# cg-tuwien/ppsurf

Hardware: AMD Instinct MI355X
Metric: occupancy query-points/sec @ res=257, 50NN (higher is better)
Workload: dtype f16x3

## Files before the change

### ppsurf_amd/csrc/pps_common.h

```cpp
#pragma once
#include <hip/hip_runtime.h>
#include <stdint.h>

typedef float f32x4 __attribute__((ext_vector_type(4)));

#define PPS_WAVE 64
#define PPS_OK 0
#define PPS_ERR_ARG 1
#define PPS_ERR_LAUNCH 2

#define PPS_SG_MFMA 0x008
#define PPS_SG_DSREAD 0x100
#define PPS_SG_VALU 0x002

namespace pps {

__device__ __forceinline__ int lane_id() { return threadIdx.x & 63; }

template <int CTRL>
__device__ __forceinline__ float dpp_mov(float v) {
    return __builtin_bit_cast(float, __builtin_amdgcn_update_dpp(0, __builtin_bit_cast(int, v), CTRL, 0xf, 0xf, true));
}
__device__ __forceinline__ float row16_max(float v) {
    v = fmaxf(v, dpp_mov<0xB1>(v));
    v = fmaxf(v, dpp_mov<0x4E>(v));
    v = fmaxf(v, dpp_mov<0x141>(v));
    v = fmaxf(v, dpp_mov<0x140>(v));
    return v;
}
__device__ __forceinline__ float row16_sum(float v) {
    v += dpp_mov<0xB1>(v);
    v += dpp_mov<0x4E>(v);
    v += dpp_mov<0x141>(v);
    v += dpp_mov<0x140>(v);
    return v;
}

__device__ __forceinline__ float max_raw(float a, float b) {
    float r;
    asm("v_max_f32 %0, %1, %2" : "=v"(r) : "v"(a), "v"(b));
    return r;
}

#define PPS_DPP4(OP, CTRL)                                                    \
    OP " %0, %0, %0 " CTRL " row_mask:0xf bank_mask:0xf bound_ctrl:1\n\t"      \
    OP " %1, %1, %1 " CTRL " row_mask:0xf bank_mask:0xf bound_ctrl:1\n\t"      \
    OP " %2, %2, %2 " CTRL " row_mask:0xf bank_mask:0xf bound_ctrl:1\n\t"      \
    OP " %3, %3, %3 " CTRL " row_mask:0xf bank_mask:0xf bound_ctrl:1\n\t"
__device__ __forceinline__ void row16_max4(float& a, float& b, float& c, float& d) {
    asm("s_nop 1\n\t" PPS_DPP4("v_max_f32_dpp", "quad_perm:[1,0,3,2]") PPS_DPP4("v_max_f32_dpp", "quad_perm:[2,3,0,1]")
        PPS_DPP4("v_max_f32_dpp", "row_half_mirror") PPS_DPP4("v_max_f32_dpp", "row_mirror")
        : "+v"(a), "+v"(b), "+v"(c), "+v"(d));
}
__device__ __forceinline__ void row16_sum4(float& a, float& b, float& c, float& d) {
    asm("s_nop 1\n\t" PPS_DPP4("v_add_f32_dpp", "quad_perm:[1,0,3,2]") PPS_DPP4("v_add_f32_dpp", "quad_perm:[2,3,0,1]")
        PPS_DPP4("v_add_f32_dpp", "row_half_mirror") PPS_DPP4("v_add_f32_dpp", "row_mirror")
        : "+v"(a), "+v"(b), "+v"(c), "+v"(d));
}
#undef PPS_DPP4

template <int CTRL>
__device__ __forceinline__ unsigned dpp_mov_u32(unsigned v) { return (unsigned)__builtin_amdgcn_update_dpp(0, (int)v, CTRL, 0xf, 0xf, true); }
__device__ __forceinline__ unsigned lane_xor_u32(unsigned v, int st, int lane) {
    switch (st) {
    case 1: return dpp_mov_u32<0xB1>(v);
    case 2: return dpp_mov_u32<0x4E>(v);
    case 4: return dpp_mov_u32<0x1B>(dpp_mov_u32<0x141>(v));
    case 8: return dpp_mov_u32<0x141>(dpp_mov_u32<0x140>(v));
    case 16: { const auto r = __builtin_amdgcn_permlane16_swap(v, v, false, false); return (lane & 16) ? r[0] : r[1]; }
    case 32: { const auto r = __builtin_amdgcn_permlane32_swap(v, v, false, false); return (lane & 32) ? r[0] : r[1]; }
    default: return (unsigned)__shfl_xor((int)v, st);
    }
}
__device__ __forceinline__ unsigned long long lane_xor_u64(unsigned long long v, int st, int lane) {
    return ((unsigned long long)lane_xor_u32((unsigned)(v >> 32), st, lane) << 32) | lane_xor_u32((unsigned)v, st, lane);
}

template <int CTRL>
__device__ __forceinline__ f32x4 dpp_mov4(f32x4 v) { return f32x4{dpp_mov<CTRL>(v.x), dpp_mov<CTRL>(v.y), dpp_mov<CTRL>(v.z), dpp_mov<CTRL>(v.w)}; }

template <int HALF, int CTRL>
__device__ __forceinline__ void butterfly_step(f32x4* v, bool upper) {
#pragma unroll
    for (int b = 0; b < HALF; ++b) {
        const f32x4 keep = upper ? v[b + HALF] : v[b];
        const f32x4 send = upper ? v[b] : v[b + HALF];
        v[b] = keep + dpp_mov4<CTRL>(send);
    }
}
__device__ __forceinline__ void rows16_sum_transposed(f32x4 (&v)[16], int lane) {
    butterfly_step<8, 0x128>(v, (lane & 8) != 0);
    butterfly_step<4, 0x141>(v, (lane & 4) != 0);
    butterfly_step<2, 0x4E>(v, (lane & 2) != 0);
// ... 209 lines not shown
template <int NF4, int NTHREADS>
__device__ __forceinline__ void chunk_copy_async(const f32x4* __restrict__ src, f32x4* dst) {
    unsigned lane_off = threadIdx.x * 16u;
    asm volatile("" : "+v"(lane_off));
    const int wave_base = threadIdx.x & ~63;
    const char* sbase = (const char*)src;
    asm volatile("" : "+s"(sbase));
#pragma unroll
    for (int i = 0; i < NF4; ++i) {
        f32x4* d = dst + i * NTHREADS + wave_base;
        const unsigned lds_addr = __builtin_amdgcn_readfirstlane((unsigned)(uintptr_t)d);
        const char* piece = sbase + (size_t)(i * NTHREADS * 16);
        asm volatile("s_mov_b32 m0, %0\n\tglobal_load_lds_dwordx4 %1, %2" : : "s"(lds_addr), "v"(lane_off), "s"(piece) : "memory", "m0");
    }
}
template <int NTHREADS>
__device__ __forceinline__ void chunk_copy_piece(const f32x4* __restrict__ src, f32x4* dst, int i) {
    unsigned lane_off = threadIdx.x * 16u;
    asm volatile("" : "+v"(lane_off));
    const int wave_base = threadIdx.x & ~63;
    const char* piece = (const char*)src + (size_t)i * (NTHREADS * 16);
    asm volatile("" : "+s"(piece));
    const unsigned lds_addr = __builtin_amdgcn_readfirstlane((unsigned)(uintptr_t)(dst + i * NTHREADS + wave_base));
    asm volatile("s_mov_b32 m0, %0\n\tglobal_load_lds_dwordx4 %1, %2" : : "s"(lds_addr), "v"(lane_off), "s"(piece) : "memory", "m0");
}
template <int NTHREADS, int NPIECES>
__device__ __forceinline__ void stream_lane_offsets(unsigned (&voff)[NPIECES]) {
#pragma unroll
    for (int i = 0; i < NPIECES; ++i) {
        voff[i] = threadIdx.x * 16u + (unsigned)i * (NTHREADS * 16u);
        asm volatile("" : "+v"(voff[i]));
    }
}
template <int NTHREADS>
__device__ __forceinline__ void chunk_copy_piece_at(const char* chunk, f32x4* dst, int i, unsigned voff) {
    const int wave_base = threadIdx.x & ~63;
    const unsigned lds_addr = __builtin_amdgcn_readfirstlane((unsigned)(uintptr_t)(dst + i * NTHREADS + wave_base));
    asm volatile("s_mov_b32 m0, %0\n\tglobal_load_lds_dwordx4 %1, %2" : : "s"(lds_addr), "v"(voff), "s"(chunk) : "memory", "m0");
}
__device__ __forceinline__ void stream_wait() {
    asm volatile("s_waitcnt vmcnt(0)" : : : "memory");
}

__device__ __forceinline__ void xcd_tile_range(int ntiles, int& first, int& count, int& stride) {
    const int nwg = gridDim.x;
    const int b = blockIdx.x;
    if ((nwg & 7) != 0 || nwg < 8) { first = b; stride = nwg; count = (ntiles > b) ? (ntiles - b + nwg - 1) / nwg : 0; return; }
    const int xcd = b & 7, slot = b >> 3, per = nwg >> 3;
    const int lo = (int)(((int64_t)ntiles * xcd) / 8), hi = (int)(((int64_t)ntiles * (xcd + 1)) / 8);
    first = lo + slot; stride = per;
    count = (hi - lo > slot) ? (hi - lo - slot + per - 1) / per : 0;
}

}
```

### ppsurf_amd/csrc/pps_decode.hip

```cpp
#include <cstdlib>
#include "pps_common.h"
#include "../../include/ppsurf_amd.h"

using namespace pps;

#ifndef NT
#define NT 256
#endif
#define NW (NT / 64)
#ifndef WG_PER_CU
#define WG_PER_CU (512 / NT)
#endif
#ifndef PPS_PRIO
#define PPS_PRIO 1
#endif
#ifndef PPS_PRIO_PN
#define PPS_PRIO_PN 1
#endif
#define CH4 2048

template <int CHUNK_F4_NEXT, int NTH = NT, class F>
__device__ __forceinline__ void stream_step(const f32x4* __restrict__ gnext, f32x4*& cur, f32x4*& nxt, F&& compute) {
    chunk_copy_async<CHUNK_F4_NEXT / NTH, NTH>(gnext, nxt);
    compute((const f32x4*)cur);
// ... 178 lines not shown
                    e[bb * 4 + r] = ev;
                    m4[bb][r] = mx;
                    s4[bb][r] = row16_sum(ev);
                }
            if (n < 4) {
                const f32x4 mm = (n == 0) ? m4[0] : (n == 1) ? m4[1] : (n == 2) ? m4[2] : m4[3];
                const f32x4 ss = (n == 0) ? s4[0] : (n == 1) ? s4[1] : (n == 2) ? s4[2] : s4[3];
                ((f32x4*)(msm + wave * 64))[4 * n + g] = mm;
                ((f32x4*)(mss + wave * 64))[4 * n + g] = ss;
            }
        }
        __syncthreads();
        {
            float mw[4], sw[4];
#pragma unroll
            for (int w2 = 0; w2 < 4; ++w2) { mw[w2] = msm[(wbase + w2) * 64 + lane]; sw[w2] = mss[(wbase + w2) * 64 + lane]; }
            const float M = fmaxf(fmaxf(mw[0], mw[1]), fmaxf(mw[2], mw[3]));
            float S = 0.f;
#pragma unroll
            for (int w2 = 0; w2 < 4; ++w2) S += sw[w2] * __expf(mw[w2] - M);
            f_l[wave * 64 + lane] = __expf(mw[wq] - M) / (64.f * S);
        }
        __syncthreads();
        float an = 0.f;
#pragma unroll
        for (int bb = 0; bb < 4; ++bb) {
            const f32x4 f4 = ((const f32x4*)(f_l + wave * 64))[4 * bb + g];
#pragma unroll
            for (int r = 0; r < 4; ++r) an += e[bb * 4 + r] * f4[r];
        }
        an += __shfl_xor(an, 16);
        an += __shfl_xor(an, 32);
#pragma unroll
        for (int bb = 0; bb < 16; ++bb) a[bb] *= an;
        rows16_sum_transposed(a, lane);
        ((f32x4*)(part + wave * 256))[4 * n + g] = a[0];
        __syncthreads();
        if (wq == 0 && qv) {
            f32x4 s = ((const f32x4*)(part + (wbase + 0) * 256))[lane];
            s += ((const f32x4*)(part + (wbase + 1) * 256))[lane];
            s += ((const f32x4*)(part + (wbase + 2) * 256))[lane];
            s += ((const f32x4*)(part + (wbase + 3) * 256))[lane];
            ((f32x4*)(pooled + qi * 256))[lane] = s;
        }
    }
}

#define IH_NT 512
#define IH_OB 2
#define IH_NW (IH_NT / 64)
#define IH_WG_PER_CU (512 / IH_NT)
#define IH_CH4 (CH4 * IH_OB / 2)
#define IH_NCH (32 / IH_OB + 4 / IH_OB)
#define IH_LDS_BYTES (2 * IH_CH4 * 16 + (IP_W_XYZ + IP_NBIAS + IH_NW * 64 * 3 + IH_NW * 256) * 4)

__global__ __launch_bounds__(IH_NT, 2) void interp_pool_f16x3_kernel(const float* __restrict__ G, const float* __restrict__ pts,
                                                                     const float* __restrict__ query, const int64_t* __restrict__ idx,
                                                                     int64_t Q, int k, const float* __restrict__ wxyz,
                                                                     const f32x4* __restrict__ w16, const float* __restrict__ bias,
                                                                     float* __restrict__ pooled, int* __restrict__ range) {
    float amax = 0.f;
    f32x4* buf0 = (f32x4*)pps_smem;
    f32x4* buf1 = buf0 + IH_CH4;
    float* xyz_l = (float*)(buf1 + IH_CH4);
    float* bias_l = xyz_l + IP_W_XYZ;
    float* msm = bias_l + IP_NBIAS;
    float* mss = msm + IH_NW * 64;
    float* f_l = mss + IH_NW * 64;
    float* part = f_l + IH_NW * 64;
    const f32x4* bias4 = (const f32x4*)bias_l;
    const f32x4* wg = w16;
    const int lane = lane_id(), wave = threadIdx.x >> 6, n = lane & 15, g = lane >> 4;

    lds_fill(xyz_l, wxyz, IP_W_XYZ);
    lds_fill(bias_l, bias, IP_NBIAS);
    stream_prologue<IH_CH4, IH_NT>(wg, buf0);
    stream_wait();
    __syncthreads();
    f32x4 *cur = buf0, *nxt = buf1;
    unsigned voff[IH_CH4 / IH_NT];
    stream_lane_offsets<IH_NT>(voff);
    const char* const wfirst = (const char*)wg;
    const char* snext = wfirst + (size_t)IH_CH4 * 16;

    const int ntiles = (int)((Q + IH_NW / 4 - 1) / (IH_NW / 4));
    int first, count, stride;
    xcd_tile_range(ntiles, first, count, stride);
    const int wq = wave & 3, wbase = wave & ~3;
    for (int it = 0; it < count; ++it) {
        const int64_t qi = (int64_t)(first + it * stride) * (IH_NW / 4) + (wave >> 2);
        const bool qv = qi < Q;
        const int64_t qc = qv ? qi : Q - 1;
        const int row = wq * 16 + n;
        const bool valid = row < k;
        const int64_t i = idx[qc * k + (valid ? row : 0)];

        HiLo x[8], y[8];
        {
            f32x4 a[16];
            const f32x4* grow = (const f32x4*)(G + i * 256) + g;
#pragma unroll
            for (int bb = 0; bb < 16; ++bb) a[bb] = grow[4 * bb];
            const float coord = (g < 3) ? (query[qc * 3 + g] - pts[i * 3 + g]) : 0.f;
            xyz_blocks<16>(coord, a, xyz_l, lane);
            relu_blocks<16>(a);
#pragma unroll
            for (int kb = 0; kb < 8; ++kb) x[kb] = split_f16_r(amax, a[2 * kb], a[2 * kb + 1]);
        }
        __builtin_amdgcn_s_setprio(PPS_PRIO);
#ifndef PPS_FCQ_PRODUCTS
#define PPS_FCQ_PRODUCTS 3
#endif
#define IH_STEP(LAST, IN, BIAS, ACTV, SINK) IH_STEP_NP(LAST, IN, BIAS, ACTV, SINK, 3)
#define IH_STEP_NP(LAST, IN, BIAS, ACTV, SINK, NPR)                                                                                   \
        {                                                                                                                             \
            stream_step_spread_at<IH_CH4, IH_NT>(snext, voff, cur, nxt, [&](const f32x4* w, auto&& piece) {                            \
                dense_blocks_f16x3_hook<8, IH_OB, ACTV, true, false, NPR>(IN, (const half8*)w, BIAS, lane, SINK,                       \
                                                    [&](int ob, int kb) { if (ob == 0 && (kb & 1) == 0) piece(kb >> 1); if (IH_CH4 / IH_NT > 4 && ob == 0 && (kb & 1)) piece(4 + (kb >> 1)); }); }); \
            snext = (LAST) ? wfirst : snext + (size_t)IH_CH4 * 16;                                                                     \
            asm volatile("" : "+s"(snext));                                      \
        }
#pragma unroll
        for (int c = 0; c < 16 / IH_OB; ++c)
            IH_STEP(false, x, bias4 + 4 * IH_OB * c, 1, ([&](int p, const f32x4& o0, const f32x4& o1) { y[IH_OB / 2 * c + p] = split_f16_r(amax, o0, o1); }));
#pragma unroll
        for (int c = 0; c < 16 / IH_OB; ++c)
            IH_STEP(false, y, bias4 + 64 + 4 * IH_OB * c, 1, ([&](int p, const f32x4& o0, const f32x4& o1) { x[IH_OB / 2 * c + p] = split_f16_r(amax, o0, o1); }));
        f32x4 b[4];
#pragma unroll
        for (int c = 0; c < 4 / IH_OB; ++c)
            IH_STEP_NP(c + 32 / IH_OB + 2 == IH_NCH, x, bias4 + 128 + 4 * IH_OB * c, 0,
                       ([&](int p, const f32x4& o0, const f32x4& o1) { b[IH_OB * c + 2 * p] = o0; b[IH_OB * c + 2 * p + 1] = o1; }), PPS_FCQ_PRODUCTS);
#undef IH_STEP
#undef IH_STEP_NP
        __builtin_amdgcn_s_setprio(0);
        float e[16];
        {
            f32x4 m4[4], s4[4];
#pragma unroll
            for (int bb = 0; bb < 4; ++bb) {
                float v[4], mx[4], sm[4];
#pragma unroll
                for (int r = 0; r < 4; ++r) mx[r] = v[r] = valid ? b[bb][r] : -INFINITY;
                row16_max4(mx[0], mx[1], mx[2], mx[3]);
#pragma unroll
                for (int r = 0; r < 4; ++r) {
                    const float ev = valid ? __expf(v[r] - mx[r]) : 0.f;
                    e[bb * 4 + r] = ev;
                    sm[r] = ev;
                }
                row16_sum4(sm[0], sm[1], sm[2], sm[3]);
                m4[bb] = f32x4{mx[0], mx[1], mx[2], mx[3]};
                s4[bb] = f32x4{sm[0], sm[1], sm[2], sm[3]};
            }
            if (n < 4) {
                const f32x4 mm = (n == 0) ? m4[0] : (n == 1) ? m4[1] : (n == 2) ? m4[2] : m4[3];
                const f32x4 ss = (n == 0) ? s4[0] : (n == 1) ? s4[1] : (n == 2) ? s4[2] : s4[3];
                ((f32x4*)(msm + wave * 64))[4 * n + g] = mm;
                ((f32x4*)(mss + wave * 64))[4 * n + g] = ss;
            }
        }
        __syncthreads();
        {
            float mw[4], sw[4];
#pragma unroll
            for (int w2 = 0; w2 < 4; ++w2) { mw[w2] = msm[(wbase + w2) * 64 + lane]; sw[w2] = mss[(wbase + w2) * 64 + lane]; }
            const float M = fmaxf(fmaxf(mw[0], mw[1]), fmaxf(mw[2], mw[3]));
            float S = 0.f;
#pragma unroll
            for (int w2 = 0; w2 < 4; ++w2) S += sw[w2] * __expf(mw[w2] - M);
            f_l[wave * 64 + lane] = __expf(mw[wq] - M) / (64.f * S);
        }
        __syncthreads();
        float an = 0.f;
#pragma unroll
        for (int bb = 0; bb < 4; ++bb) {
            const f32x4 f4 = ((const f32x4*)(f_l + wave * 64))[4 * bb + g];
#pragma unroll
            for (int r = 0; r < 4; ++r) an += e[bb * 4 + r] * f4[r];
        }
        an += __shfl_xor(an, 16);
        an += __shfl_xor(an, 32);
        f32x4 a[16];
#pragma unroll
        for (int kb = 0; kb < 8; ++kb) {
            join_f16(x[kb], a[2 * kb], a[2 * kb + 1]);
            a[2 * kb] *= an;
            a[2 * kb + 1] *= an;
        }
        rows16_sum_transposed(a, lane);
        ((f32x4*)(part + wave * 256))[4 * n + g] = a[0];
        __syncthreads();
        if (wq == 0 && qv) {
            f32x4 s = ((const f32x4*)(part + (wbase + 0) * 256))[lane];
            s += ((const f32x4*)(part + (wbase + 1) * 256))[lane];
            s += ((const f32x4*)(part + (wbase + 2) * 256))[lane];
            s += ((const f32x4*)(part + (wbase + 3) * 256))[lane];
            ((f32x4*)(pooled + qi * 256))[lane] = s;
        }
    }
    range_commit(amax, range);
}

#define IS_NT 256
#define IS_MAX_OUT 8
template <int CB, bool H>
__global__ __launch_bounds__(IS_NT) void interp_small_kernel(const float* __restrict__ G, const float* __restrict__ pts,
                                                             const float* __restrict__ query, const int64_t* __restrict__ idx,
                                                             int64_t Q, int k, const float* __restrict__ wpack, const float* __restrict__ w16,
                                                             const float* __restrict__ bias, const float* __restrict__ wtail, int nout,
                                                             float* __restrict__ out, int* __restrict__ guard) {
    constexpr int C = 16 * CB, NWX = 64 * CB, NW2 = 256 * CB * CB, NWQ = 1024 * CB, NB = 2 * C + 64, KB = CB / 2;
    if (!H) {
        if (gate_closed(guard)) return;
        if (guard != nullptr && blockIdx.x == 0 && threadIdx.x == 0) atomicAdd(guard + 1, 1);
    }
    float amax = 0.f;
    __shared__ __attribute__((aligned(16))) float lds[NWX + 2 * NW2 + NWQ + NB + 4 * 64 * 3 + 4 * C + IS_MAX_OUT * (C + 1)];
    float* xyz_l = lds;
    const f32x4* w2 = (const f32x4*)(lds + NWX);
    const f32x4* w3 = (const f32x4*)(lds + NWX + NW2);
    const f32x4* wq = (const f32x4*)(lds + NWX + 2 * NW2);
    float* bias_l = lds + NWX + 2 * NW2 + NWQ;
    float* msm = bias_l + NB;
    float* mss = msm + 256;
    float* f_l = mss + 256;
// ... 174 lines not shown
        dense_blocks_f16x3<2, 4, 1>(b, (const half8*)w, bias4 + 32, lane, [&](int i, const f32x4& o0, const f32x4& o1) { a[i] = split_f16_r(amax, o0, o1); }); });
#pragma unroll
    for (int h = 0; h < PN_C2N; ++h)
        stream_step<PCH4, PNT>(wg + 2048 + (h + 1) * PCH4, cur, nxt, [&](const f32x4* w) {
            dense_blocks_f16x3<2, PN_C2OB, 1>(a, (const half8*)w, bias4 + 48 + 4 * PN_C2OB * h, lane,
                                              [&](int i, const f32x4& o0, const f32x4& o1) { y[PN_C2OB / 2 * h + i] = split_f16_r(amax, o0, o1); }); });
#pragma unroll
    for (int c = 0; c < PN_C3N - 1; ++c)
        stream_step<PCH4, PNT>(wg + 4096 + (c + 1) * PCH4, cur, nxt, [&](const f32x4* w) {
            dense_blocks_f16x3<4, PN_C3OB, 1>(y, (const half8*)w, bias4 + 80 + 4 * PN_C3OB * c, lane,
                                              [&](int i, const f32x4& o0, const f32x4& o1) { z[PN_C3OB * c + 2 * i] = o0; z[PN_C3OB * c + 2 * i + 1] = o1; }); });
    stream_step<1024, PNT>(wg, cur, nxt, [&](const f32x4* w) {
        dense_blocks_f16x3<4, PN_C3OB, 1>(y, (const half8*)w, bias4 + 80 + 4 * PN_C3OB * (PN_C3N - 1), lane,
                                          [&](int i, const f32x4& o0, const f32x4& o1) { z[PN_C3OB * (PN_C3N - 1) + 2 * i] = o0; z[PN_C3OB * (PN_C3N - 1) + 2 * i + 1] = o1; }); });
    __builtin_amdgcn_s_setprio(0);
}

template <int T, class ZSink>
__device__ __forceinline__ void stn_chain_h_tiles(const float (&coord)[T], const float* xyz_l, const f32x4* bias4, const f32x4* wg,
                                                  f32x4*& cur, f32x4*& nxt, int lane, float& amax, ZSink&& zsink) {
    const int g = lane >> 4;
    HiLo a[T][2], b[T][2], y[T][4];
#pragma unroll
    for (int t = 0; t < T; ++t) {
        f32x4 x0[4];
#pragma unroll
        for (int bb = 0; bb < 4; ++bb) x0[bb] = bias4[4 * bb + g];
        xyz_blocks<4>(coord[t], x0, xyz_l, lane);
        relu_blocks<4>(x0);
        a[t][0] = split_f16_r(amax, x0[0], x0[1]);
        a[t][1] = split_f16_r(amax, x0[2], x0[3]);
    }
    __builtin_amdgcn_s_setprio(PPS_PRIO_PN);
    stream_step<1024, PNT>(wg + 1024, cur, nxt, [&](const f32x4* w) {
        dense_blocks_f16x3_tiles<T, 2, 4, 1>(a, (const half8*)w, bias4 + 16, lane, [&](int t, int i, const f32x4& o0, const f32x4& o1) { b[t][i] = split_f16_r(amax, o0, o1); }); });
    stream_step<PCH4, PNT>(wg + 2048, cur, nxt, [&](const f32x4* w) {
        dense_blocks_f16x3_tiles<T, 2, 4, 1>(b, (const half8*)w, bias4 + 32, lane, [&](int t, int i, const f32x4& o0, const f32x4& o1) { a[t][i] = split_f16_r(amax, o0, o1); }); });
#pragma unroll
    for (int h = 0; h < PN_C2N; ++h)
        stream_step<PCH4, PNT>(wg + 2048 + (h + 1) * PCH4, cur, nxt, [&](const f32x4* w) {
            dense_blocks_f16x3_tiles<T, 2, PN_C2OB, 1>(a, (const half8*)w, bias4 + 48 + 4 * PN_C2OB * h, lane,
                                                      [&](int t, int i, const f32x4& o0, const f32x4& o1) { y[t][PN_C2OB / 2 * h + i] = split_f16_r(amax, o0, o1); }); });
#pragma unroll
    for (int c = 0; c < PN_C3N - 1; ++c)
        stream_step<PCH4, PNT>(wg + 4096 + (c + 1) * PCH4, cur, nxt, [&](const f32x4* w) {
            dense_blocks_f16x3_tiles<T, 4, PN_C3OB, 1>(y, (const half8*)w, bias4 + 80 + 4 * PN_C3OB * c, lane,
                                                      [&](int t, int i, const f32x4& o0, const f32x4& o1) { zsink(t, PN_C3OB * c + 2 * i, o0, o1); }); });
    stream_step<1024, PNT>(wg, cur, nxt, [&](const f32x4* w) {
        dense_blocks_f16x3_tiles<T, 4, PN_C3OB, 1>(y, (const half8*)w, bias4 + 80 + 4 * PN_C3OB * (PN_C3N - 1), lane,
                                                  [&](int t, int i, const f32x4& o0, const f32x4& o1) { zsink(t, PN_C3OB * (PN_C3N - 1) + 2 * i, o0, o1); }); });
    __builtin_amdgcn_s_setprio(0);
}

template <bool H>
__global__ __launch_bounds__(PNT, 2) void pointnet_stn_rows_kernel(const float* __restrict__ patches, int64_t Q, int P, int pack,
                                                                   const float* __restrict__ wpack, const f32x4* __restrict__ wdense,
                                                                   const float* __restrict__ bias, float* __restrict__ gout, int* __restrict__ flag) {
    if (!H && gate_closed(flag)) return;
    float amax = 0.f;
    f32x4* buf0 = (f32x4*)pps_smem;
    f32x4* buf1 = buf0 + PCH4;
    float* xyz_l = (float*)(buf1 + PCH4);
    float* bias_l = xyz_l + PA_W_XYZ;
    float* park = bias_l + PA_NBIAS;
    const f32x4* bias4 = (const f32x4*)bias_l;
    const f32x4* wg = wdense;
    const int lane = lane_id(), wave = threadIdx.x >> 6, n = lane & 15, g = lane >> 4;
    float* mypark = park + wave * PN_PARK_ROWS * PN_ROWF;

    lds_fill(xyz_l, wpack, PA_W_XYZ);
    lds_fill(bias_l, bias, PA_NBIAS);
    stream_prologue<1024, PNT>(wg, buf0);
    stream_wait();
    __syncthreads();
    f32x4 *cur = buf0, *nxt = buf1;

    const PatchPacking pk = patch_packing(P, pack);
    const int64_t ngroups = (Q + pk.qg - 1) / pk.qg;
    const int ntiles = (int)((ngroups + PNW - 1) / PNW);
    int first, count, stride;
    xcd_tile_range(ntiles, first, count, stride);
    for (int it = 0; it < count; ++it) {
        const int64_t q0 = ((int64_t)(first + it * stride) * PNW + wave) * pk.qg;
        if constexpr (H) {
            if (pk.packed) {
                const int ql = n / pk.lo;
                const int64_t qq = (q0 + ql < Q) ? q0 + ql : Q - 1;
                const float coord[1] = {(g < 3) ? patches[(qq * P + pk.fb * 16 + (n % pk.lo)) * 3 + g] : 0.f};
                stn_chain_h_tiles<1>(coord, xyz_l, bias4, wg, cur, nxt, lane, amax, [&](int, int bb, const f32x4& o0, const f32x4& o1) {
                    f32x4 m0, m1;
#pragma unroll
                    for (int r = 0; r < 4; ++r) { m0[r] = group_max(o0[r], pk.lo); m1[r] = group_max(o1[r], pk.lo); }
                    if ((n % pk.lo) == 0) { ((f32x4*)(mypark + ql * PN_ROWF))[4 * bb + g] = m0; ((f32x4*)(mypark + ql * PN_ROWF))[4 * (bb + 1) + g] = m1; }
                });
            }
            for (int qi = 0; qi < pk.qg; ++qi) {
                const int64_t q = q0 + qi;
                const bool qv = q < Q;
                const int64_t qc = qv ? q : Q - 1;
                f32x4 rmax[16];
#pragma unroll
                for (int bb = 0; bb < 16; ++bb)
                    rmax[bb] = pk.packed ? ((const f32x4*)(mypark + qi * PN_ROWF))[4 * bb + g] : f32x4{-INFINITY, -INFINITY, -INFINITY, -INFINITY};
                auto zmax = [&](int, int bb, const f32x4& o0, const f32x4& o1) {
#pragma unroll
                    for (int r = 0; r < 4; ++r) { rmax[bb][r] = max_raw(rmax[bb][r], o0[r]); rmax[bb + 1][r] = max_raw(rmax[bb + 1][r], o1[r]); }
                };
                auto row_coord = [&](int rb) {
                    const int row = rb * 16 + n;
                    const int rowc = row < P ? row : P - 1;
                    return (g < 3) ? patches[(qc * P + rowc) * 3 + g] : 0.f;
                };
                int rb = 0;
                for (; rb + 1 < pk.fb; rb += 2) {
                    const float coord[2] = {row_coord(rb), row_coord(rb + 1)};
                    stn_chain_h_tiles<2>(coord, xyz_l, bias4, wg, cur, nxt, lane, amax, zmax);
                }
                if (rb < pk.fb) {
                    const float coord[1] = {row_coord(rb)};
                    stn_chain_h_tiles<1>(coord, xyz_l, bias4, wg, cur, nxt, lane, amax, zmax);
                }
#pragma unroll
                for (int bb = 0; bb < 16; ++bb) {
                    float p0 = rmax[bb][0], p1 = rmax[bb][1], p2 = rmax[bb][2], p3 = rmax[bb][3];
                    row16_max4(p0, p1, p2, p3);
                    if (n == 0 && qv) ((f32x4*)(gout + q * 256))[4 * bb + g] = f32x4{p0, p1, p2, p3};
                }
            }
            continue;
        }
        f32x4 z[16];
        if (pk.packed) {
            const int ql = n / pk.lo;
            const int64_t qq = (q0 + ql < Q) ? q0 + ql : Q - 1;
            const float coord = (g < 3) ? patches[(qq * P + pk.fb * 16 + (n % pk.lo)) * 3 + g] : 0.f;
            if (H) stn_chain_h(coord, z, xyz_l, bias4, wg, cur, nxt, lane, amax); else stn_chain(coord, z, xyz_l, bias4, wg, cur, nxt, lane);
#pragma unroll
            for (int bb = 0; bb < 16; ++bb) {
                f32x4 m;
#pragma unroll
                for (int r = 0; r < 4; ++r) m[r] = group_max(z[bb][r], pk.lo);
                if ((n % pk.lo) == 0) ((f32x4*)(mypark + ql * PN_ROWF))[4 * bb + g] = m;
            }
        }
        for (int qi = 0; qi < pk.qg; ++qi) {
            const int64_t q = q0 + qi;
            const bool qv = q < Q;
// ... 549 lines not shown
        }
    }
    range_commit(amax, range);
}

static int g_cu_count = 0;
static int cu_count() {
    if (g_cu_count == 0) {
        int dev = 0;
        hipDeviceProp_t prop;
        if (hipGetDevice(&dev) != hipSuccess || hipGetDeviceProperties(&prop, dev) != hipSuccess) return -1;
        g_cu_count = prop.multiProcessorCount;
    }
    return g_cu_count;
}

template <class K>
static int set_lds(K kernel, int bytes) {
    return hipFuncSetAttribute((const void*)kernel, hipFuncAttributeMaxDynamicSharedMemorySize, bytes) == hipSuccess ? 0 : 1;
}

static int grid_for(int64_t ntiles) {
    int cus = cu_count();
    if (cus <= 0) cus = 256;
    cus *= WG_PER_CU;
    return (int)(ntiles < cus ? (ntiles > 0 ? ntiles : 1) : cus);
}

struct PnSplit { int64_t q_packed; int grid_packed, grid_rest, rest_mode; };
static PnSplit pn_split(int64_t q, int p) {
    int cus = cu_count();
    if (cus <= 0) cus = 256;
    const PatchPacking pk = patch_packing(p);
    PnSplit sp;
    const int wgs = cus * PN_WG_PER_CU;
    const int64_t per_round = (int64_t)wgs * PNW * pk.qg;
    sp.q_packed = pk.packed ? (q / per_round) * per_round : 0;
    if (pk.packed && getenv("PPS_PN_FORCE_PACK")) sp.q_packed = q;
    sp.grid_packed = wgs;
    sp.rest_mode = pk.packed ? 2 : 0;
    const int64_t rest_tiles = (q - sp.q_packed + PNW - 1) / PNW;
    sp.grid_rest = (int)(rest_tiles < wgs ? rest_tiles : wgs);
    return sp;
}

#define PPS_LAUNCH_CHECK() (hipGetLastError() == hipSuccess ? PPS_OK : PPS_ERR_LAUNCH)

template <bool H>
static int launch_stn_rows(const float* patches, int64_t q, int p, const float* wpack, const void* wdense, const float* bias, float* g,
                           int* flag, void* stream) {
    static int once = set_lds(pointnet_stn_rows_kernel<H>, PA_LDS_BYTES);
    (void)once;
    const PnSplit sp = pn_split(q, p);
    if (sp.q_packed > 0)
        hipLaunchKernelGGL(pointnet_stn_rows_kernel<H>, dim3(sp.grid_packed), dim3(PNT), PA_LDS_BYTES, (hipStream_t)stream, patches,
                           sp.q_packed, p, 1, wpack, (const f32x4*)wdense, bias, g, flag);
    if (q > sp.q_packed)
        hipLaunchKernelGGL(pointnet_stn_rows_kernel<H>, dim3(sp.grid_rest), dim3(PNT), PA_LDS_BYTES, (hipStream_t)stream,
                           patches + sp.q_packed * p * 3, q - sp.q_packed, p, sp.rest_mode, wpack, (const f32x4*)wdense, bias, g + sp.q_packed * 256, flag);
    return PPS_LAUNCH_CHECK();
}

template <bool H>
static int launch_feat_rows(const float* patches, const float* trans2, int64_t q, int p, const float* wpack, const void* wdense,
                            const float* bias, float* xbar, int* flag, void* stream) {
    static int once = set_lds(pointnet_feat_rows_kernel<H>, PC_LDS_BYTES);
    (void)once;
    int cus = cu_count();
    if (cus <= 0) cus = 256;
    const int64_t ntiles = (q + PNW - 1) / PNW, wgs = (int64_t)cus * PN_WG_PER_CU;
    hipLaunchKernelGGL(pointnet_feat_rows_kernel<H>, dim3((unsigned)(ntiles < wgs ? ntiles : wgs)), dim3(PNT), PC_LDS_BYTES, (hipStream_t)stream, patches,
                       trans2, q, p, wpack, (const f32x4*)wdense, bias, xbar, flag);
    return PPS_LAUNCH_CHECK();
}


static int interp_pool_f32_impl(const float* G, const float* pts, const float* query, const int64_t* idx, int64_t q, int k,
                                const float* wpack, const float* bias, float* pooled, const int* gate, void* stream) {
    if (q < 0 || k < 1 || k > 64) return PPS_ERR_ARG;
    if (q == 0) return PPS_OK;
    if (!G || !pts || !query || !idx || !wpack || !bias || !pooled) return PPS_ERR_ARG;
    static int once = set_lds(interp_pool_kernel, IP_LDS_BYTES);
    (void)once;
    hipLaunchKernelGGL(interp_pool_kernel, dim3(grid_for((q + NW / 4 - 1) / (NW / 4))), dim3(NT), IP_LDS_BYTES, (hipStream_t)stream,
                       G, pts, query, idx, q, k, wpack, bias, pooled, gate);
    return PPS_LAUNCH_CHECK();
}

static int stn_fc_f32_impl(const float* g, int64_t q, const float* wpack, const float* bias, float* trans2, const int* gate, void* stream) {
    if (q < 0) return PPS_ERR_ARG;
    if (q == 0) return PPS_OK;
    if (!g || !wpack || !bias || !trans2) return PPS_ERR_ARG;
    static int once = set_lds(pointnet_stn_fc_kernel, PB_LDS_BYTES);
    (void)once;
    hipLaunchKernelGGL(pointnet_stn_fc_kernel, dim3(grid_for((q + NW * 16 * PB_T - 1) / (NW * 16 * PB_T))), dim3(NT), PB_LDS_BYTES, (hipStream_t)stream,
                       g, q, wpack, bias, trans2, gate);
    return PPS_LAUNCH_CHECK();
}

static int decode_tail_f32_impl(const float* pooled, const float* xbar, int64_t q, const float* wpack, const float* bias,
                                float* logits, float* occ, int* gate, void* stream) {
    if (q < 0) return PPS_ERR_ARG;
    if (q == 0) return PPS_OK;
    if (!pooled || !xbar || !wpack || !bias || !logits) return PPS_ERR_ARG;
    static int once = set_lds(decode_tail_kernel, TL_LDS_BYTES);
    (void)once;
    hipLaunchKernelGGL(decode_tail_kernel, dim3(grid_for((q + NW * 16 - 1) / (NW * 16))), dim3(NT), TL_LDS_BYTES, (hipStream_t)stream,
                       pooled, xbar, q, wpack, bias, logits, occ, gate);
    return PPS_LAUNCH_CHECK();
}

extern "C" {

int pps_abi_version(void) { return 2; }

int pps_debug_occupancy(int which) {
    int n = -1;
    if (which == 0) { set_lds(interp_pool_kernel, IP_LDS_BYTES); hipOccupancyMaxActiveBlocksPerMultiprocessor(&n, interp_pool_kernel, NT, IP_LDS_BYTES); }
    if (which == 1) { set_lds(pointnet_stn_rows_kernel<false>, PA_LDS_BYTES); hipOccupancyMaxActiveBlocksPerMultiprocessor(&n, pointnet_stn_rows_kernel<false>, PNT, PA_LDS_BYTES); }
    if (which == 3) { set_lds(pointnet_stn_fc_kernel, PB_LDS_BYTES); hipOccupancyMaxActiveBlocksPerMultiprocessor(&n, pointnet_stn_fc_kernel, NT, PB_LDS_BYTES); }
    if (which == 4) { set_lds(pointnet_stn_fc_h_kernel, PB_LDS_BYTES); hipOccupancyMaxActiveBlocksPerMultiprocessor(&n, pointnet_stn_fc_h_kernel, NT, PB_LDS_BYTES); }
    if (which == 2) { set_lds(pointnet_feat_rows_kernel<false>, PC_LDS_BYTES); hipOccupancyMaxActiveBlocksPerMultiprocessor(&n, pointnet_feat_rows_kernel<false>, PNT, PC_LDS_BYTES); }
    return n;
}
int pps_device_cu_count(void) { return cu_count(); }

int pps_rows_dense256_f32(const float* in, int64_t rs, int64_t cs, int64_t m, const float* wpack, const float* bias,
                          float* out, void* stream) {
    if (m < 0) return PPS_ERR_ARG;
    if (m == 0) return PPS_OK;
    if (!in || !wpack || !bias || !out) return PPS_ERR_ARG;
    if (cs == 1 && (rs % 4) != 0) return PPS_ERR_ARG;
    static int once = set_lds(rows_dense256_kernel, RD_LDS_BYTES);
    (void)once;
    hipLaunchKernelGGL(rows_dense256_kernel, dim3(grid_for((m + NW * 16 - 1) / (NW * 16))), dim3(NT), RD_LDS_BYTES, (hipStream_t)stream,
                       in, rs, cs, m, wpack, bias, out);
    return PPS_LAUNCH_CHECK();
}

int pps_interp_pool_f32(const float* G, const float* pts, const float* query, const int64_t* idx, int64_t q, int k,
                        const float* wpack, const float* bias, float* pooled, void* stream) {
    return interp_pool_f32_impl(G, pts, query, idx, q, k, wpack, bias, pooled, nullptr, stream);
}

int pps_interp_pool_f16x3(const float* G, const float* pts, const float* query, const int64_t* idx, int64_t q, int k,
                          const float* wxyz, const void* w16, const float* bias, float* pooled, int32_t* range_flag, void* stream) {
    if (q < 0 || k < 1 || k > 64) return PPS_ERR_ARG;
    if (q == 0) return PPS_OK;
    if (!G || !pts || !query || !idx || !wxyz || !w16 || !bias || !pooled) return PPS_ERR_ARG;
    static int once = set_lds(interp_pool_f16x3_kernel, IH_LDS_BYTES);
    (void)once;
    int cus = cu_count();
    if (cus <= 0) cus = 256;
    const int64_t ntiles = (q + IH_NW / 4 - 1) / (IH_NW / 4);
    const int64_t wgs = (int64_t)cus * IH_WG_PER_CU;
    const int grid = (int)(ntiles < wgs ? ntiles : wgs);
    hipLaunchKernelGGL(interp_pool_f16x3_kernel, dim3(grid), dim3(IH_NT), IH_LDS_BYTES, (hipStream_t)stream,
                       G, pts, query, idx, q, k, wxyz, (const f32x4*)w16, bias, pooled, (int*)range_flag);
    return PPS_LAUNCH_CHECK();
}

int pps_interp_small_f32(const float* G, const float* pts, const float* query, const int64_t* idx, int64_t q, int k, int c,
                         const float* wpack, const float* bias, const float* wtail, int nout, float* out, void* stream) {
    if (q < 0 || k < 1 || k > 64 || (c != 32 && c != 64) || nout < 1 || nout > IS_MAX_OUT) return PPS_ERR_ARG;
    if (q == 0) return PPS_OK;
    if (!G || !pts || !query || !idx || !wpack || !bias || !wtail || !out) return PPS_ERR_ARG;
    int cus = cu_count();
    if (cus <= 0) cus = 256;
    const int grid = (int)(q < (int64_t)cus * 8 ? q : (int64_t)cus * 8);
    hipStream_t st = (hipStream_t)stream;
    if (c == 32) hipLaunchKernelGGL((interp_small_kernel<2, false>), dim3(grid), dim3(IS_NT), 0, st, G, pts, query, idx, q, k, wpack, nullptr, bias, wtail, nout, out, nullptr);
    else hipLaunchKernelGGL((interp_small_kernel<4, false>), dim3(grid), dim3(IS_NT), 0, st, G, pts, query, idx, q, k, wpack, nullptr, bias, wtail, nout, out, nullptr);
    return PPS_LAUNCH_CHECK();
}

int pps_interp_small_f16x3(const float* G, const float* pts, const float* query, const int64_t* idx, int64_t q, int k, int c,
                           const float* wpack, const void* w16, const float* bias, const float* wtail, int nout, float* out, int* guard,
                           void* stream) {
    if (q < 0 || k < 1 || k > 64 || (c != 32 && c != 64) || nout < 1 || nout > IS_MAX_OUT) return PPS_ERR_ARG;
    if (q == 0) return PPS_OK;
    if (!G || !pts || !query || !idx || !wpack || !w16 || !bias || !wtail || !out || !guard) return PPS_ERR_ARG;
    int cus = cu_count();
    if (cus <= 0) cus = 256;
    const int grid = (int)(q < (int64_t)cus * 8 ? q : (int64_t)cus * 8);
    hipStream_t st = (hipStream_t)stream;
    if (hipMemsetAsync(guard, 0, sizeof(int), st) != hipSuccess) return PPS_ERR_LAUNCH;
    const float* wh = (const float*)w16;
    if (c == 32) {
        hipLaunchKernelGGL((interp_small_kernel<2, true>), dim3(grid), dim3(IS_NT), 0, st, G, pts, query, idx, q, k, wpack, wh, bias, wtail, nout, out, guard);
        hipLaunchKernelGGL((interp_small_kernel<2, false>), dim3(grid), dim3(IS_NT), 0, st, G, pts, query, idx, q, k, wpack, nullptr, bias, wtail, nout, out, guard);
    } else {
        hipLaunchKernelGGL((interp_small_kernel<4, true>), dim3(grid), dim3(IS_NT), 0, st, G, pts, query, idx, q, k, wpack, wh, bias, wtail, nout, out, guard);
        hipLaunchKernelGGL((interp_small_kernel<4, false>), dim3(grid), dim3(IS_NT), 0, st, G, pts, query, idx, q, k, wpack, nullptr, bias, wtail, nout, out, guard);
    }
    return PPS_LAUNCH_CHECK();
}

int pps_pointnet_stn_rows_f32(const float* patches, int64_t q, int p, const float* wpack, const float* bias, float* g,
                              void* stream) {
    if (q < 0 || p < 1) return PPS_ERR_ARG;
    if (q == 0) return PPS_OK;
    if (!patches || !wpack || !bias || !g) return PPS_ERR_ARG;
    return launch_stn_rows<false>(patches, q, p, wpack, wpack + PA_W_XYZ, bias, g, nullptr, stream);
}

int pps_pointnet_stn_fc_f32(const float* g, int64_t q, const float* wpack, const float* bias, float* trans2, void* stream) {
    return stn_fc_f32_impl(g, q, wpack, bias, trans2, nullptr, stream);
}

int pps_pointnet_feat_rows_f32(const float* patches, const float* trans2, int64_t q, int p, const float* wpack,
                               const float* bias, float* xbar, void* stream) {
// ... 147 lines not shown
```

Before: 13.01 million.

## Keep final head weights resident in LDS and use wave-level sync for softmax

Adds a templated variant of the f16x3 interp-pool kernel that copies the final head (fcq) weight chunks into LDS once per workgroup. The per-query stream then wraps around after the second dense layer instead of streaming those chunks every tile. This cuts global weight traffic and stream steps per query but raises LDS use per workgroup, which could lower occupancy. It also swaps a block-wide __syncthreads for a per-wave LDS wait plus wave barrier before reading f_l. An env var can select the old path; the resident variant is the default.

```diff
diff --git a/ppsurf_amd/csrc/pps_common.h b/ppsurf_amd/csrc/pps_common.h
--- a/ppsurf_amd/csrc/pps_common.h
+++ b/ppsurf_amd/csrc/pps_common.h
@@ -354,4 +354,9 @@
     count = (hi - lo > slot) ? (hi - lo - slot + per - 1) / per : 0;
 }
 
-}
+__device__ __forceinline__ void lds_wave_sync() {
+    asm volatile("s_waitcnt lgkmcnt(0)" : : : "memory");
+    __builtin_amdgcn_wave_barrier();
+}
+
+}
diff --git a/ppsurf_amd/csrc/pps_decode.hip b/ppsurf_amd/csrc/pps_decode.hip
--- a/ppsurf_amd/csrc/pps_decode.hip
+++ b/ppsurf_amd/csrc/pps_decode.hip
@@ -254,8 +254,10 @@
 #define IH_WG_PER_CU (512 / IH_NT)
 #define IH_CH4 (CH4 * IH_OB / 2)
 #define IH_NCH (32 / IH_OB + 4 / IH_OB)
-#define IH_LDS_BYTES (2 * IH_CH4 * 16 + (IP_W_XYZ + IP_NBIAS + IH_NW * 64 * 3 + IH_NW * 256) * 4)
-
+#define IH_FCQ4 (4 / IH_OB * IH_CH4)
+#define IH_LDS_BYTES(RES) (2 * IH_CH4 * 16 + (IP_W_XYZ + IP_NBIAS + IH_NW * 64 * 3 + IH_NW * 256) * 4 + ((RES) ? IH_FCQ4 * 16 : 0))
+
+template <bool RES>
 __global__ __launch_bounds__(IH_NT, 2) void interp_pool_f16x3_kernel(const float* __restrict__ G, const float* __restrict__ pts,
                                                                      const float* __restrict__ query, const int64_t* __restrict__ idx,
                                                                      int64_t Q, int k, const float* __restrict__ wxyz,
@@ -270,6 +272,7 @@
     float* mss = msm + IH_NW * 64;
     float* f_l = mss + IH_NW * 64;
     float* part = f_l + IH_NW * 64;
+    f32x4* fcq_l = (f32x4*)(part + IH_NW * 256);
     const f32x4* bias4 = (const f32x4*)bias_l;
     const f32x4* wg = w16;
     const int lane = lane_id(), wave = threadIdx.x >> 6, n = lane & 15, g = lane >> 4;
@@ -277,6 +280,10 @@
     lds_fill(xyz_l, wxyz, IP_W_XYZ);
     lds_fill(bias_l, bias, IP_NBIAS);
     stream_prologue<IH_CH4, IH_NT>(wg, buf0);
+    if constexpr (RES) {
+        const f32x4* src = wg + (size_t)(32 / IH_OB) * IH_CH4;
+        for (int i = threadIdx.x; i < IH_FCQ4; i += IH_NT) fcq_l[i] = src[i];
+    }
     stream_wait();
     __syncthreads();
     f32x4 *cur = buf0, *nxt = buf1;
@@ -327,12 +334,18 @@
             IH_STEP(false, x, bias4 + 4 * IH_OB * c, 1, ([&](int p, const f32x4& o0, const f32x4& o1) { y[IH_OB / 2 * c + p] = split_f16_r(amax, o0, o1); }));
 #pragma unroll
         for (int c = 0; c < 16 / IH_OB; ++c)
-            IH_STEP(false, y, bias4 + 64 + 4 * IH_OB * c, 1, ([&](int p, const f32x4& o0, const f32x4& o1) { x[IH_OB / 2 * c + p] = split_f16_r(amax, o0, o1); }));
+            IH_STEP(RES && c + 16 / IH_OB + 2 == 32 / IH_OB, y, bias4 + 64 + 4 * IH_OB * c, 1,
+                    ([&](int p, const f32x4& o0, const f32x4& o1) { x[IH_OB / 2 * c + p] = split_f16_r(amax, o0, o1); }));
         f32x4 b[4];
 #pragma unroll
-        for (int c = 0; c < 4 / IH_OB; ++c)
-            IH_STEP_NP(c + 32 / IH_OB + 2 == IH_NCH, x, bias4 + 128 + 4 * IH_OB * c, 0,
-                       ([&](int p, const f32x4& o0, const f32x4& o1) { b[IH_OB * c + 2 * p] = o0; b[IH_OB * c + 2 * p + 1] = o1; }), PPS_FCQ_PRODUCTS);
+        for (int c = 0; c < 4 / IH_OB; ++c) {
+            auto heads = [&](int p, const f32x4& o0, const f32x4& o1) { b[IH_OB * c + 2 * p] = o0; b[IH_OB * c + 2 * p + 1] = o1; };
+            if constexpr (RES)
+                dense_blocks_f16x3_hook<8, IH_OB, 0, true, false, PPS_FCQ_PRODUCTS>(x, (const half8*)(fcq_l + c * IH_CH4), bias4 + 128 + 4 * IH_OB * c, lane,
+                                                                                   heads, [](int, int) {});
+            else
+                IH_STEP_NP(c + 32 / IH_OB + 2 == IH_NCH, x, bias4 + 128 + 4 * IH_OB * c, 0, heads, PPS_FCQ_PRODUCTS);
+        }
 #undef IH_STEP
 #undef IH_STEP_NP
         __builtin_amdgcn_s_setprio(0);
@@ -373,7 +386,7 @@
             for (int w2 = 0; w2 < 4; ++w2) S += sw[w2] * __expf(mw[w2] - M);
             f_l[wave * 64 + lane] = __expf(mw[wq] - M) / (64.f * S);
         }
-        __syncthreads();
+        lds_wave_sync();
         float an = 0.f;
 #pragma unroll
         for (int bb = 0; bb < 4; ++bb) {
@@ -1446,15 +1459,20 @@
     if (q < 0 || k < 1 || k > 64) return PPS_ERR_ARG;
     if (q == 0) return PPS_OK;
     if (!G || !pts || !query || !idx || !wxyz || !w16 || !bias || !pooled) return PPS_ERR_ARG;
-    static int once = set_lds(interp_pool_f16x3_kernel, IH_LDS_BYTES);
+    static int once = set_lds(interp_pool_f16x3_kernel<true>, IH_LDS_BYTES(true)) | set_lds(interp_pool_f16x3_kernel<false>, IH_LDS_BYTES(false));
     (void)once;
     int cus = cu_count();
     if (cus <= 0) cus = 256;
     const int64_t ntiles = (q + IH_NW / 4 - 1) / (IH_NW / 4);
     const int64_t wgs = (int64_t)cus * IH_WG_PER_CU;
     const int grid = (int)(ntiles < wgs ? ntiles : wgs);
-    hipLaunchKernelGGL(interp_pool_f16x3_kernel, dim3(grid), dim3(IH_NT), IH_LDS_BYTES, (hipStream_t)stream,
-                       G, pts, query, idx, q, k, wxyz, (const f32x4*)w16, bias, pooled, (int*)range_flag);
+    const char* res_env = getenv("PPS_IP_FCQ_RESIDENT");
+    if (res_env && res_env[0] == '0' && res_env[1] == 0)
+        hipLaunchKernelGGL(interp_pool_f16x3_kernel<false>, dim3(grid), dim3(IH_NT), IH_LDS_BYTES(false), (hipStream_t)stream,
+                           G, pts, query, idx, q, k, wxyz, (const f32x4*)w16, bias, pooled, (int*)range_flag);
+    else
+        hipLaunchKernelGGL(interp_pool_f16x3_kernel<true>, dim3(grid), dim3(IH_NT), IH_LDS_BYTES(true), (hipStream_t)stream,
+                           G, pts, query, idx, q, k, wxyz, (const f32x4*)w16, bias, pooled, (int*)range_flag);
     return PPS_LAUNCH_CHECK();
 }
 
```

New measurement: 13.09 million (median of 6 runs). About the same (+0.6%).

## Process all STN row tiles of a query in one weight-streaming pass

Applied to the files above, without the earlier changes.

Adds a one-pass path to the STN rows kernel. When the patch needs at most three 16-row tiles, all tiles of a query go through the dense chain together, so the streamed weights are read once per query instead of once per tile. The per-tile outputs are combined with v_max3 and a DPP row reduction, then stored directly. This trades more live registers (several tiles of activations held at once) for fewer weight-stream passes, and the path can be limited to two tiles via an environment variable.

```diff
diff --git a/ppsurf_amd/csrc/pps_common.h b/ppsurf_amd/csrc/pps_common.h
--- a/ppsurf_amd/csrc/pps_common.h
+++ b/ppsurf_amd/csrc/pps_common.h
@@ -39,6 +39,11 @@
 __device__ __forceinline__ float max_raw(float a, float b) {
     float r;
     asm("v_max_f32 %0, %1, %2" : "=v"(r) : "v"(a), "v"(b));
+    return r;
+}
+__device__ __forceinline__ float max3_raw(float a, float b, float c) {
+    float r;
+    asm("v_max3_f32 %0, %1, %2, %3" : "=v"(r) : "v"(a), "v"(b), "v"(c));
     return r;
 }
 
diff --git a/ppsurf_amd/csrc/pps_decode.hip b/ppsurf_amd/csrc/pps_decode.hip
--- a/ppsurf_amd/csrc/pps_decode.hip
+++ b/ppsurf_amd/csrc/pps_decode.hip
@@ -654,8 +654,47 @@
     __builtin_amdgcn_s_setprio(0);
 }
 
+template <int T>
+__device__ __forceinline__ void stn_query_tiles(const float* __restrict__ qpatch, int P, const float* prow, float* gq, bool store, const float* xyz_l,
+                                                const f32x4* bias4, const f32x4* wg, f32x4*& cur, f32x4*& nxt, int lane, float& amax) {
+    const int n = lane & 15, g = lane >> 4;
+    float coord[T];
+#pragma unroll
+    for (int t = 0; t < T; ++t) {
+        const int row = t * 16 + n;
+        const int rowc = row < P ? row : P - 1;
+        coord[t] = (g < 3) ? qpatch[rowc * 3 + g] : 0.f;
+    }
+    f32x4 h0[T], h1[T];
+    stn_chain_h_tiles<T>(coord, xyz_l, bias4, wg, cur, nxt, lane, amax, [&](int t, int bb, const f32x4& o0, const f32x4& o1) {
+        h0[t] = o0; h1[t] = o1;
+        if (t != T - 1) return;
+        const f32x4 k0 = ((const f32x4*)prow)[4 * bb + g], k1 = ((const f32x4*)prow)[4 * (bb + 1) + g];
+        float p[4], s[4];
+#pragma unroll
+        for (int r = 0; r < 4; ++r) {
+            if constexpr (T == 3) {
+                p[r] = max_raw(max3_raw(h0[0][r], h0[1][r], h0[2][r]), k0[r]);
+                s[r] = max_raw(max3_raw(h1[0][r], h1[1][r], h1[2][r]), k1[r]);
+            } else if constexpr (T == 2) {
+                p[r] = max3_raw(h0[0][r], h0[1][r], k0[r]);
+                s[r] = max3_raw(h1[0][r], h1[1][r], k1[r]);
+            } else {
+                p[r] = max_raw(h0[0][r], k0[r]);
+                s[r] = max_raw(h1[0][r], k1[r]);
+            }
+        }
+        row16_max4(p[0], p[1], p[2], p[3]);
+        row16_max4(s[0], s[1], s[2], s[3]);
+        if (n == 0 && store) {
+            ((f32x4*)gq)[4 * bb + g] = f32x4{p[0], p[1], p[2], p[3]};
+            ((f32x4*)gq)[4 * (bb + 1) + g] = f32x4{s[0], s[1], s[2], s[3]};
+        }
+    });
+}
+
 template <bool H>
-__global__ __launch_bounds__(PNT, 2) void pointnet_stn_rows_kernel(const float* __restrict__ patches, int64_t Q, int P, int pack,
+__global__ __launch_bounds__(PNT, 2) void pointnet_stn_rows_kernel(const float* __restrict__ patches, int64_t Q, int P, int pack, int tmax,
                                                                    const float* __restrict__ wpack, const f32x4* __restrict__ wdense,
                                                                    const float* __restrict__ bias, float* __restrict__ gout, int* __restrict__ flag) {
     if (!H && gate_closed(flag)) return;
@@ -680,6 +719,9 @@
     const PatchPacking pk = patch_packing(P, pack);
     const int64_t ngroups = (Q + pk.qg - 1) / pk.qg;
     const int ntiles = (int)((ngroups + PNW - 1) / PNW);
+    const bool one_pass = H && tmax >= 3 && pk.fb <= 3;
+    if (one_pass && !pk.packed)
+        for (int i = lane; i < PN_ROWF; i += 64) mypark[i] = -INFINITY;
     int first, count, stride;
     xcd_tile_range(ntiles, first, count, stride);
     for (int it = 0; it < count; ++it) {
@@ -695,6 +737,19 @@
                     for (int r = 0; r < 4; ++r) { m0[r] = group_max(o0[r], pk.lo); m1[r] = group_max(o1[r], pk.lo); }
                     if ((n % pk.lo) == 0) { ((f32x4*)(mypark + ql * PN_ROWF))[4 * bb + g] = m0; ((f32x4*)(mypark + ql * PN_ROWF))[4 * (bb + 1) + g] = m1; }
                 });
+            }
+            if (one_pass) {
+                for (int qi = 0; qi < pk.qg; ++qi) {
+                    const int64_t q = q0 + qi;
+                    const bool qv = q < Q;
+                    const float* qpatch = patches + (qv ? q : Q - 1) * P * 3;
+                    const float* prow = mypark + qi * PN_ROWF;
+                    float* gq = gout + (qv ? q : 0) * 256;
+                    if (pk.fb == 3) stn_query_tiles<3>(qpatch, P, prow, gq, qv, xyz_l, bias4, wg, cur, nxt, lane, amax);
+                    else if (pk.fb == 2) stn_query_tiles<2>(qpatch, P, prow, gq, qv, xyz_l, bias4, wg, cur, nxt, lane, amax);
+                    else stn_query_tiles<1>(qpatch, P, prow, gq, qv, xyz_l, bias4, wg, cur, nxt, lane, amax);
+                }
+                continue;
             }
             for (int qi = 0; qi < pk.qg; ++qi) {
                 const int64_t q = q0 + qi;
@@ -1350,12 +1405,15 @@
     static int once = set_lds(pointnet_stn_rows_kernel<H>, PA_LDS_BYTES);
     (void)once;
     const PnSplit sp = pn_split(q, p);
+    const char* tiles_env = getenv("PPS_STN_TILES");
+    const int tmax = (tiles_env && atoi(tiles_env) == 2) ? 2 : 3;
     if (sp.q_packed > 0)
         hipLaunchKernelGGL(pointnet_stn_rows_kernel<H>, dim3(sp.grid_packed), dim3(PNT), PA_LDS_BYTES, (hipStream_t)stream, patches,
-                           sp.q_packed, p, 1, wpack, (const f32x4*)wdense, bias, g, flag);
+                           sp.q_packed, p, 1, tmax, wpack, (const f32x4*)wdense, bias, g, flag);
     if (q > sp.q_packed)
         hipLaunchKernelGGL(pointnet_stn_rows_kernel<H>, dim3(sp.grid_rest), dim3(PNT), PA_LDS_BYTES, (hipStream_t)stream,
-                           patches + sp.q_packed * p * 3, q - sp.q_packed, p, sp.rest_mode, wpack, (const f32x4*)wdense, bias, g + sp.q_packed * 256, flag);
+                           patches + sp.q_packed * p * 3, q - sp.q_packed, p, sp.rest_mode, tmax, wpack, (const f32x4*)wdense, bias,
+                           g + sp.q_packed * 256, flag);
     return PPS_LAUNCH_CHECK();
 }
 
```

Measured after the change: 13.03 million before, 13.21 million after, median of 6. 1.4% higher.
